# AmnonDrory/LidarRegistration

Hardware: AMD Instinct MI355X
Metric: registration pairs/sec (30k-pt FCGF pairs, mutual-NN + 50k RANSAC iters + refit) (higher is better)
Workload: dtype f32; 1 GPU; configs[1]: 30000-pt x32-d synthetic FCGF pair, --mode MNN --iters 50000, 3-pt sampling + ELC + LS refit; 192 distinct resident pairs per GPU, T copied to the host inside the timed region; pairs_per_batched_call=32, batched_calls_in_flight_per_gpu=2, parallelism=pair-sharded x1

## Files before the change

### lidarregistration_amd/csrc/lr_api.hip

```cpp
#include "lr_internal.h"
#include <stdarg.h>
#include <string.h>
#include <stdlib.h>
#include <new>

static thread_local char g_err[512] = "";

void lr_set_error(const char *fmt, ...)
{
    va_list ap;
    va_start(ap, fmt);
    vsnprintf(g_err, sizeof(g_err), fmt, ap);
    va_end(ap);
}

static_assert(sizeof(lr_ransac_params) == 72 && sizeof(lr_pair_params) == 112 && sizeof(lr_pair_result) == 496,
              "ABI structs changed: update include/lidarreg.h, _ext.py, INTEGRATION.md and tests/test_abi_cpu.py together");

extern "C" int lr_version(void) { return 103; }
extern "C" const char *lr_last_error(void) { return g_err; }

static inline void forget_last_batch(lr_workspace *ws) { if (ws) { ws->last_batch = 0; ws->last_T_final = nullptr; } }

static int g_fake_device = -1;
// ... 77 lines not shown
        T *p = base ? reinterpret_cast<T *>(base + off) : nullptr;
        off += sizeof(T) * count;
        return p;
    }
};

void carve(lr_workspace *ws, Carver &c)
{
    const size_t n0 = ws->max_n0, n1 = ws->max_n1, n = ws->max_n, it = ws->max_iters;
    ws->nrm0 = c.take<float>(n0); ws->nrm1 = c.take<float>(n1);
    ws->H0 = c.take<_Float16>(n0 * 32); ws->H1 = c.take<_Float16>(n1 * 32);
    if (ws->dim != LR_FEAT_DIM) { ws->P0 = c.take<float>(n0 * 32); ws->P1 = c.take<float>(n1 * 32); }
    ws->tau = c.take<float>(n);
    ws->yfin = c.take<float>(n * LR_NN_MAX_STRIPS);
    ws->yshare = c.take<uint32_t>(n);
    ws->cand_cnt = c.take<int32_t>(LR_NN16_CNT_INTS(n)); ws->cand = c.take<int32_t>(LR_NN16_SEG_INTS(n));
    ws->counters = c.take<int32_t>(LR_CNT_TOTAL);
    ws->bmax0 = c.take<float>(n0 / 32 + 2); ws->bmax1 = c.take<float>(n1 / 32 + 2);
    ws->bmin0 = c.take<float>(n0 / 32 + 2); ws->bmin1 = c.take<float>(n1 / 32 + 2);
    ws->nn_range = c.take<float>(8);
    ws->rev_seed = c.take<uint32_t>(n1); ws->rev_rows = c.take<int32_t>(n1);
    ws->rev_seed64 = c.take<unsigned long long>(n1);
    ws->rev_cols = c.take<int32_t>(n0); ws->rev_s1 = c.take<float>(n0); ws->rev_pos = c.take<int32_t>(n0);
    ws->rev_tmin = c.take<float>(n0 / 32 + 2); ws->rev_hist = c.take<int32_t>(2 * 4096);
    ws->Hs = c.take<_Float16>(n0 * 32); ws->nrms = c.take<float>(n0);
    ws->nn_idx1 = c.take<int32_t>(n0); ws->nn_idx2 = c.take<int32_t>(n0);
    ws->nn_s1 = c.take<float>(n0); ws->nn_s2 = c.take<float>(n0);
    ws->rev_idx1 = c.take<int32_t>(n1);
    ws->is_bb = c.take<uint8_t>(n0);
    ws->blk_cnt = c.take<int32_t>(n0 / 256 + 2);
    ws->corr_idx0 = c.take<int32_t>(n0); ws->corr_idx1 = c.take<int32_t>(n0); ws->corr_idx2 = c.take<int32_t>(n0);
    ws->corr_score = c.take<float>(n0);
    ws->ratio = c.take<float>(n0);
    ws->cell = c.take<int32_t>(n0); ws->cell_sorted = c.take<int32_t>(n0);
    ws->gpf_quota = c.take<double>(LR_GPF_MAX_CELLS);
    ws->gpf_cells = c.take<int32_t>(3 * (LR_GPF_MAX_CELLS + 8) > 2 * (LR_PR_BUCKETS + 8) + 8 ? 3 * (LR_GPF_MAX_CELLS + 8) : 2 * (LR_PR_BUCKETS + 8) + 8);
    ws->gpf_keep = c.take<uint8_t>(n0);
    ws->gpf_f = c.take<float>(8);
    ws->corr8 = c.take<float>((n0 + 2) * 8);
    ws->prosac_G = c.take<int32_t>(n0 + 2); ws->prosac_rank = c.take<int32_t>(n0);
    ws->models = c.take<float>(it * 12);
    ws->models64 = c.take<double>(it * 12);
    ws->model_h = c.take<int32_t>(it);
    ws->models2 = c.take<float>(it * 12); ws->models64_2 = c.take<double>(it * 12); ws->model_h2 = c.take<int32_t>(it);
    ws->score_cnt = c.take<uint32_t>(it);
    ws->score_ssq = c.take<unsigned long long>(it);
    ws->refit_part = c.take<double>((n0 / 256 + 2) * 16);
// ... 157 lines not shown
__global__ void __launch_bounds__(256) zero_scratch_kernel(uint32_t *__restrict__ p, size_t words, lr_zargs z)
{
    lr_z(p, z, blockIdx.z);
    for (size_t k = (size_t)blockIdx.x * 256 + threadIdx.x; k < words; k += (size_t)gridDim.x * 256) p[k] = 0u;
}
int lr_zero_scratch(const lr_call &c, void *p, size_t bytes)
{
    const size_t words = (bytes + 3) / 4;
    int blocks = (int)((words + 255) / 256);
    if (blocks > 1024) blocks = 1024;
    hipLaunchKernelGGL(zero_scratch_kernel, dim3(blocks < 1 ? 1 : blocks, 1, c.pairs), dim3(256), 0, c.st, reinterpret_cast<uint32_t *>(p), words, c.z);
    LR_LAUNCH_CHECK();
    return LR_OK;
}

extern "C" int lr_workspace_clock(lr_workspace *ws, double *mhz, unsigned long long *cycles, unsigned long long *ticks, int reset)
{
    LR_CHECK_DEVICE(ws, nullptr, "lr_workspace_clock");
    unsigned long long h[2] = { 0ull, 0ull };
    LR_HIP(hipMemcpy(h, ws->clk_dev, sizeof h, hipMemcpyDeviceToHost));
    if (cycles) *cycles = h[0];
    if (ticks) *ticks = h[1];
    if (mhz) *mhz = h[1] ? 100.0 * (double)h[0] / (double)h[1] : 0.0;
    if (reset) LR_HIP(hipMemset(ws->clk_dev, 0, sizeof h));
    return LR_OK;
}

int lr_timer_mark(const lr_call &c, lr_event e)
{
    lr_stage_timer &t = c.ws->timer;
    bool due = false;
    switch (e) {
    case LR_EV_FWD_FILTER_BEGIN: case LR_EV_FWD_FILTER_END: due = c.armed && !t.begun(); break;
    case LR_EV_REV_FILTER_BEGIN: case LR_EV_REV_FILTER_END: due = t.begun() && !t.has(LR_EV_REV_FILTER_END) && !t.has(LR_EV_RANSAC_END); break;
    case LR_EV_RANSAC_BEGIN: case LR_EV_RANSAC_END: due = t.begun() && !t.has(LR_EV_RANSAC_END); break;
    case LR_EV_CALL_BEGIN: case LR_EV_FWD_NN_DONE: case LR_EV_REV_NN_DONE: due = c.armed; break;
    case LR_EV_CALL_END: due = c.armed && t.has(LR_EV_RANSAC_END); break;
    case LR_NEV: break;
    }
    if (!t.on || !due) return LR_OK;
    LR_HIP(hipEventRecord(t.ev[e], c.st));
    t.recorded |= 1u << e;
    return LR_OK;
}

static int lr_timer_collect(lr_stage_timer &t)
{
// ... 359 lines not shown
```

### lidarregistration_amd/csrc/lr_internal.h

```cpp
#pragma once
#include <hip/hip_runtime.h>
#include <stdint.h>
#include <stdio.h>
#include "../../include/lidarreg.h"

void lr_set_error(const char *fmt, ...);

#define LR_HIP(call)                                                                      \
    do {                                                                                  \
        hipError_t e_ = (call);                                                           \
        if (e_ != hipSuccess) {                                                           \
            lr_set_error("%s:%d: %s -> %s", __FILE__, __LINE__, #call, hipGetErrorString(e_)); \
            return LR_EHIP;                                                               \
        }                                                                                 \
    } while (0)

#define LR_LAUNCH_CHECK() LR_HIP(hipGetLastError())

#define LR_REQUIRE(cond, code, msg)                 \
    do {                                            \
        if (!(cond)) { lr_set_error("%s", msg); return code; } \
    } while (0)

#define LR_NN16_SEG 4096
// ... 13 lines not shown
        } } while (0)

#define LR_NN_MAX_STRIPS 8
#define LR_FEAT_DIM 32

#ifndef LR_SCORE_BLOCKS
#define LR_SCORE_BLOCKS 2048
#endif
#define LR_GPF_MAX_CELLS 4096
#define LR_PR_BUCKETS 8192
#define LR_SC_INFO_BYTES 2048
#define LR_LO_CTL_BYTES 20480

struct lr_pair_desc {
    const float *xyz0, *xyz1, *F0, *F1;
    int32_t n0, n1;
};
struct lr_zargs {
    size_t stride;
    const lr_pair_desc *descs;
};
#define LR_MAX_BATCH 64
struct lr_desc_table { lr_pair_desc d[LR_MAX_BATCH]; };

#ifdef __HIPCC__
#define lr_z(p, z, pair) \
    do { const size_t lr_zo_ = (size_t)(pair) * (z).stride; p = (decltype(p))((const char *)(p) + (lr_zo_ & ((size_t)0 - (size_t)((p) != nullptr)))); } while (0)
__device__ __forceinline__ bool lr_xcd_block(int total, int &logical)
{
    const int chunk = (int)gridDim.x >> 3;
    logical = ((int)blockIdx.x & 7) * chunk + ((int)blockIdx.x >> 3);
    return logical < total;
}
#endif

enum lr_event {
    LR_EV_FWD_FILTER_BEGIN, LR_EV_FWD_FILTER_END,
    LR_EV_RANSAC_BEGIN, LR_EV_RANSAC_END,
    LR_EV_REV_FILTER_BEGIN, LR_EV_REV_FILTER_END,
    LR_EV_CALL_BEGIN,
    LR_EV_FWD_NN_DONE, LR_EV_CALL_END, LR_EV_REV_NN_DONE,
    LR_NEV
};
struct lr_stage_timer {
    int on;
    unsigned recorded;
// ... 16 lines not shown
    hipStream_t last_stream;
    size_t stride;
    size_t bytes;
    char *base;
    lr_pair_desc *descs;
    float *nrm0, *nrm1;
    _Float16 *H0, *H1;
    float *P0, *P1;
    float *tau;
    uint32_t *yshare;
    float *yfin;
    int32_t *cand_cnt, *cand;
    float *bmax0, *bmax1;
    float *bmin0, *bmin1;
    float *nn_range;
    int form_prev[2];
    int32_t *form_host, *form_dev;
    uint32_t *rev_seed;
    unsigned long long *rev_seed64;
    int32_t *rev_rows;
    int32_t *rev_cols;
    int32_t *rev_pos;
    float *rev_s1;
    float *rev_tmin;
    int32_t *rev_hist;
    _Float16 *Hs; float *nrms;
    int nn_blocks_target;
    int nn_blocks_batch;
    int nn_sample_stride;
    int rev_strips;
    int nn_second_auto;
    int clock_probe;
    unsigned long long *clk_dev;
    int32_t *counters;
    int32_t *nn_idx1, *nn_idx2;
    float *nn_s1, *nn_s2;
    int32_t *rev_idx1;
    uint8_t *is_bb;
    int32_t *blk_cnt;
    int32_t *corr_idx0, *corr_idx1, *corr_idx2;
    float *corr_score;
    float *ratio;
    int32_t *cell;
    int32_t *cell_sorted;
    double *gpf_quota;
    int32_t *gpf_cells;
    uint8_t *gpf_keep;
    float *gpf_f;
// ... 108 lines not shown
```

### lidarregistration_amd/csrc/lr_nn16.hip

```cpp
#include "lr_internal.h"
#include <math.h>
#include <stdlib.h>
#include <type_traits>

typedef float f32x4 __attribute__((ext_vector_type(4)));
typedef float f32x2 __attribute__((ext_vector_type(2)));
typedef _Float16 f16x8 __attribute__((ext_vector_type(8)));

#define LR_INF __builtin_huge_valf()
#define LR_IMAX 0x7fffffff

__device__ __forceinline__ uint32_t lr_ord_enc(float v) { const uint32_t b = __float_as_uint(v); return (b & 0x80000000u) ? ~b : (b | 0x80000000u); }
__device__ __forceinline__ float lr_ord_dec(uint32_t u) { return __uint_as_float((u & 0x80000000u) ? (u & 0x7fffffffu) : ~u); }
#define LR_ORD_INF 0xff800000u

__global__ void __launch_bounds__(256)
nn16_prep_kernel(const float *__restrict__ Fa, int na, _Float16 *__restrict__ Ha, float *__restrict__ nrma, float *__restrict__ bmaxa, float *__restrict__ bmina,
                 const float *__restrict__ Fb, int nb, _Float16 *__restrict__ Hb, float *__restrict__ nrmb, float *__restrict__ bmaxb, float *__restrict__ bminb,
                 uint32_t *__restrict__ seed_b, unsigned long long *__restrict__ seed64_b, int32_t *__restrict__ counters, int zero_counters, int nblk_a,
                 uint32_t *__restrict__ yshare_a, lr_zargs z)
{
    __shared__ float s_m[4], s_n[4];
    if (z.descs) { const lr_pair_desc d = z.descs[blockIdx.z]; Fa = d.F0; na = d.n0; Fb = d.F1; nb = d.n1; }
    lr_z(bmina, z, blockIdx.z); lr_z(bminb, z, blockIdx.z);
    lr_z(Ha, z, blockIdx.z); lr_z(nrma, z, blockIdx.z); lr_z(bmaxa, z, blockIdx.z); lr_z(Hb, z, blockIdx.z); lr_z(nrmb, z, blockIdx.z);
    lr_z(bmaxb, z, blockIdx.z); lr_z(seed_b, z, blockIdx.z); lr_z(seed64_b, z, blockIdx.z); lr_z(counters, z, blockIdx.z); lr_z(yshare_a, z, blockIdx.z);
    if (counters && blockIdx.x == 0 && (int)threadIdx.x < LR_CNT_TOTAL) {
        const int k = threadIdx.x;
// ... 158 lines not shown
        atomicMin(&o.seed_range[0], __float_as_uint(lo));
        atomicMax(&o.seed_range[1], __float_as_uint(hi));
    }
}
__device__ __forceinline__ bool ex_bad8(const f32x4 &u, const f32x4 &v)
{
    const float big = fmaxf(fmaxf(fmaxf(fabsf(u.x), fabsf(u.y)), fmaxf(fabsf(u.z), fabsf(u.w))), fmaxf(fmaxf(fabsf(v.x), fabsf(v.y)), fmaxf(fabsf(v.z), fabsf(v.w))));
    return !(big <= 65504.0f) || u.x != u.x || u.y != u.y || u.z != u.z || u.w != u.w || v.x != v.x || v.y != v.y || v.z != v.z || v.w != v.w;
}

#ifdef LR_PB_PROBE
__device__ unsigned long long lr_pb_stat[16];
#define LR_PROBE(...) __VA_ARGS__
#else
#define LR_PROBE(...)
#endif
#define LR_PB_WAVES 3
template <bool SIGN>
__global__ void __launch_bounds__(256) __attribute__((amdgpu_waves_per_eu(LR_PB_WAVES, LR_PB_WAVES)))
nn16_passb_kernel(lr_pb_tail tail_first , unsigned long long *clk_on,
                  const _Float16 *__restrict__ Hq, int na_host, const int32_t *__restrict__ rowmap, const int32_t *__restrict__ na_dev,
                  const _Float16 *__restrict__ Hc, const float *__restrict__ nC, int nb,
                  int tiles_per_strip, const float *__restrict__ tau, int32_t *__restrict__ cand_cnt, int32_t *__restrict__ cand,
                  const int32_t *__restrict__ colmap, const float *__restrict__ tile_min, const uint32_t *__restrict__ row_bound,
                  const int32_t *__restrict__ rev_offs, const uint32_t *__restrict__ rev_range, float *__restrict__ yfin, int yfin_stride,
                  uint32_t *__restrict__ yshare, int32_t *__restrict__ form_miss, lr_thr_in thr, lr_pb_grid pg, lr_zargs z)
{
    int logical;
    if (!lr_xcd_block(pg.total, logical)) return;
    const int bx = logical % pg.gx, by = (logical / pg.gx) % pg.gy, pair = logical / (pg.gx * pg.gy);
    if (z.descs) {
        const lr_pair_desc d = z.descs[pair];
        na_host = pg.dir ? d.n1 : d.n0; nb = pg.dir ? d.n0 : d.n1;
    }
    lr_z(Hq, z, pair); lr_z(rowmap, z, pair); lr_z(na_dev, z, pair); lr_z(Hc, z, pair); lr_z(nC, z, pair); lr_z(tau, z, pair);
    lr_z(cand_cnt, z, pair); lr_z(cand, z, pair); lr_z(colmap, z, pair); lr_z(tile_min, z, pair); lr_z(row_bound, z, pair); lr_z(rev_offs, z, pair); lr_z(rev_range, z, pair);
    lr_z(thr.nQ, z, pair); lr_z(thr.range_c, z, pair); lr_z(yfin, z, pair); lr_z(yshare, z, pair);
    const int na = na_dev ? *na_dev : na_host;
    if (bx * LR_BLOCK_ROWS >= na) return;
    float max_nc = 0.0f, min_nc = 0.0f;
    if (thr.range_c) { max_nc = thr.range_c[0]; min_nc = thr.range_c[1]; }
    const bool sign_ok = thr.range_c != nullptr && min_nc > 0.0f && max_nc < LR_INF && max_nc - min_nc <= 1e-4f * max_nc && true;
    if (sign_ok != SIGN) {
        if (pg.only && form_miss && bx == 0 && by == 0 && threadIdx.x == 0) { lr_z(form_miss, z, pair); *form_miss = 1; }
        return;
    }
    const float xhat = SIGN ? 0.5f * min_nc : 0.0f;
    __shared__ int s_limit[4];
    __shared__ unsigned long long s_clk[2];
    if (clk_on && threadIdx.x == 0) { s_clk[0] = __builtin_amdgcn_s_memtime(); s_clk[1] = __builtin_amdgcn_s_memrealtime(); }
    constexpr int CH = LR_PB_CH;
    constexpr int XOFF = CH * 32 * LR_LDS_ROW;
    constexpr int BUF = XOFF + (SIGN ? 0 : CH * 32 * 4);
    __shared__ __attribute__((aligned(16))) unsigned char lds_a[BUF];
    __shared__ __attribute__((aligned(16))) unsigned char lds_b[BUF];
    constexpr int WL = (LR_PB_CH >= 8 && !SIGN) ? (LR_PB_WLIST * 7) / 8 : LR_PB_WLIST;
    __shared__ uint2 wlist[4][WL];
    __shared__ __attribute__((aligned(16))) float s_Y[LR_BLOCK_ROWS];
    __shared__ float s_D[LR_BLOCK_ROWS], s_N1[LR_BLOCK_ROWS], s_N2[LR_BLOCK_ROWS];
    __shared__ unsigned s_att[2];
    const int tid = threadIdx.x, wave = __builtin_amdgcn_readfirstlane(tid >> 6), lane = tid & 63;
    const int c16 = lane & 15, kb = lane >> 4;
    const int row0 = bx * LR_BLOCK_ROWS + wave * 64;
    LR_PROBE(int n_visits = 0, n_hits = 0, n_rounds = 0, n_groups = 0, n_tk_derive = 0, n_tk_flush = 0, n_tk_a = 0, n_tk_b = 0;
             const unsigned long long tk_start = __builtin_amdgcn_s_memrealtime(); unsigned long long tk_walk = 0;)
    int ntiles = (nb + 31) >> 5;
    int my_strips = pg.gy;
    if (tile_min) {
        if (tid == 0) {
            const float lo = __uint_as_float(rev_range[0]), scale = rs_scale(lo, __uint_as_float(rev_range[1]));
            const float sv = __uint_as_float(row_bound[rowmap[bx * LR_BLOCK_ROWS]]);
            const int b = rs_bucket(sv, lo, scale);
            s_limit[0] = ((b + 1 < LR_RS_BUCKETS ? rev_offs[b + 1] : nb) + 31) >> 5;
        }
        __syncthreads();
        ntiles = min(ntiles, s_limit[0]);
        my_strips = min(pg.gy, (ntiles + tiles_per_strip - 1) / tiles_per_strip);
        if (by >= my_strips) return;
        tiles_per_strip = (ntiles + my_strips - 1) / my_strips;
    }
    const int t_begin = by * tiles_per_strip;
    const int t_end = min(ntiles, t_begin + tiles_per_strip);
    const int nchunks = t_end > t_begin ? (t_end - t_begin + CH - 1) / CH : 0;

    f16x8 a16[4];
#pragma unroll
    for (int rbk = 0; rbk < 4; ++rbk) {
        int row = min(row0 + 16 * rbk + c16, na - 1);
        if (rowmap) row = rowmap[row];
        a16[rbk] = *reinterpret_cast<const f16x8 *>(Hq + (size_t)row * 32 + 8 * kb);
    }

    f32x4 stage[CH / 2];
    float stage_n = 0.0f;

    {
        const int rw = bx * LR_BLOCK_ROWS + tid;
        float Dv = LR_INF;
        if (thr.nQ && rw < na) {
// ... 582 lines not shown
    lr_workspace *ws = c.ws;
    hipLaunchKernelGGL(nn16_prep_kernel, dim3(lr_cdiv(n0, 32) + lr_cdiv(n1, 32), 1, c.pairs), dim3(256), 0, c.st, F0, n0, ws->H0, ws->nrm0, ws->bmax0, ws->bmin0,
                       F1, n1, ws->H1, ws->nrm1, ws->bmax1, ws->bmin1, ws->rev_seed, ws->rev_seed64, ws->counters, zero_counters ? 1 : 0, lr_cdiv(n0, 32), ws->yshare, c.z);
    hipLaunchKernelGGL(nn16_range_kernel, dim3(2, 1, c.pairs), dim3(256), 0, c.st, n0, (const float *)ws->bmax0, (const float *)ws->bmin0, n1, (const float *)ws->bmax1,
                       (const float *)ws->bmin1, ws->nn_range, c.pairs == 1 ? ws->form_dev : (int32_t *)nullptr, c.z);
    LR_LAUNCH_CHECK();
    return LR_OK;
}

static int lr_nn16_form_hint(const lr_call &c, int col_cloud)
{
    lr_workspace *ws = c.ws;
    if (c.pairs != 1 || !ws->form_host) return 0;
    const int h = *reinterpret_cast<const volatile int32_t *>(&ws->form_host[col_cloud]);
    const int prev = ws->form_prev[col_cloud];
    ws->form_prev[col_cloud] = h;
    return ((h == 1 || h == 2) && h == prev) ? h : 0;
}

struct lr_pb_args {
    const _Float16 *Hq; int na; const int32_t *rowmap, *na_dev;
    const _Float16 *Hc; const float *nC; int nb, tps;
    const float *tau;
    const int32_t *colmap; const float *tile_min; const uint32_t *row_bound; const int32_t *rev_offs; const uint32_t *rev_range;
    float *yfin; int yfin_stride; uint32_t *yshare;
    lr_thr_in thr;
    int row_blocks, strips, dir;
};
static int lr_nn16_passb(const lr_call &c, const lr_pb_args &a)
{
    lr_workspace *ws = c.ws;
    const int total = a.row_blocks * a.strips * c.pairs;
    const dim3 grid(8 * lr_cdiv(total, 8));
    LR_TRY_HIP(lr_timer_mark(c, a.dir ? LR_EV_REV_FILTER_BEGIN : LR_EV_FWD_FILTER_BEGIN));
    const int only = lr_nn16_form_hint(c, a.dir ? 0 : 1);
    int32_t *miss = ws->counters + (a.dir ? LR_CNT_FORM_MISS_R : LR_CNT_FORM_MISS_F);
    unsigned long long *clk = ws->clock_probe ? ws->clk_dev : (unsigned long long *)nullptr;
    const lr_pb_tail tl = { clk };
    const lr_pb_grid pg = { a.row_blocks, a.strips, total, a.dir, only };
    auto launch = [&](auto kernel) {
        hipLaunchKernelGGL(kernel, grid, dim3(256), 0, c.st, tl, clk, a.Hq, a.na, a.rowmap, a.na_dev, a.Hc, a.nC, a.nb, a.tps, a.tau, ws->cand_cnt, ws->cand,
                           a.colmap, a.tile_min, a.row_bound, a.rev_offs, a.rev_range, a.yfin, a.yfin_stride, a.yshare, miss, a.thr, pg, c.z);
    };
    if (only != 2) launch(nn16_passb_kernel<true>);
    if (only != 1) launch(nn16_passb_kernel<false>);
    return lr_timer_mark(c, a.dir ? LR_EV_REV_FILTER_END : LR_EV_FWD_FILTER_END);
}

int lr_nn16_run(const lr_call &c, const float *Fq, int na, const float *Fc, int nb,
                int32_t *idx1, int32_t *idx2, float *s1, float *s2, bool seed_reverse)
{
    lr_workspace *ws = c.ws;
    const float *nQ = ws->nrm0, *nC = ws->nrm1, *range_c = ws->nn_range + 2;
    const int need = idx2 ? 2 : 1;
    const int ntiles = lr_cdiv(nb, 32);
    const int row_blocks = lr_cdiv(na, LR_BLOCK_ROWS);
    int strips = c.pairs > 1 ? lr_cdiv(ws->nn_blocks_batch, row_blocks * c.pairs) : ws->nn_blocks_target / row_blocks;
    int smax = ntiles / 64;
    if (strips > smax) strips = smax;
    if (strips > LR_NN_MAX_STRIPS) strips = LR_NN_MAX_STRIPS;
    if (strips < 1) strips = 1;
    const int tps = lr_cdiv(ntiles, strips);
    int sstride = ws->nn_sample_stride > 0 ? ws->nn_sample_stride : (strips > 1 ? ntiles / 64 : tps / 32);
    if (ws->nn_sample_stride <= 0) { const int cap = strips > 1 ? 16 : 32; if (sstride > cap) sstride = cap; }
    if (sstride < 1) sstride = 1;
// ... 32 lines not shown
        const f32x4 a = pa[k], b = pb[k];
        acc = __builtin_fmaf(a.x, b.x, acc);
        acc = __builtin_fmaf(a.y, b.y, acc);
        acc = __builtin_fmaf(a.z, b.z, acc);
        acc = __builtin_fmaf(a.w, b.w, acc);
    }
    const float d2 = __builtin_fmaf(-2.0f, acc, n0v[i] + n1v[j]);
    sv = __builtin_sqrtf(fmaxf(d2, 1e-30f));
    if (!(sv < 3.0e38f)) sv = 3.0e38f;
    atomicMin(&seed_bits[j], __float_as_uint(sv));
    s1[i] = sv;
    }
    float lo = i < n0 ? sv : 3.0e38f, hi = i < n0 ? sv : 0.0f;
#pragma unroll
    for (int k = 32; k >= 1; k >>= 1) { lo = fminf(lo, __shfl_xor(lo, k)); hi = fmaxf(hi, __shfl_xor(hi, k)); }
    if ((threadIdx.x & 63) == 0) { s_lo[threadIdx.x >> 6] = lo; s_hi[threadIdx.x >> 6] = hi; }
    __syncthreads();
    if (threadIdx.x == 0) {
        atomicMin(&range[0], __float_as_uint(fminf(fminf(s_lo[0], s_lo[1]), fminf(s_lo[2], s_lo[3]))));
        atomicMax(&range[1], __float_as_uint(fmaxf(fmaxf(s_hi[0], s_hi[1]), fmaxf(s_hi[2], s_hi[3]))));
    }
}

#define LR_RO_ROUND 8192
#define LR_RO_QUEUE 3072
__global__ void __launch_bounds__(1024)
nn16_rev_order_kernel(int n0, int n1, const float *__restrict__ s1, const uint32_t *__restrict__ seed_bits, const uint32_t *__restrict__ range,
                      int32_t *__restrict__ offs, int32_t *__restrict__ n_rows, const float *__restrict__ block_max_c, int nblk_c,
                      const float *__restrict__ nrm1, const _Float16 *__restrict__ H0, const float *__restrict__ nrm0, int32_t *__restrict__ colmap,
                      _Float16 *__restrict__ H0s, float *__restrict__ nrm0s, int32_t *__restrict__ rowmap, float *__restrict__ tau,
                      int32_t *__restrict__ cand_cnt, int32_t *__restrict__ rev_out, int seg_counters, lr_zargs z)
{
    __shared__ int s_pos[2 * LR_RS_BUCKETS];
    __shared__ int2 s_q[LR_RO_QUEUE];
    __shared__ float s_m[16];
    __shared__ int s_w[16], s_own[4], s_nq, s_nrows;
    if (z.descs) { n0 = z.descs[blockIdx.z].n0; n1 = z.descs[blockIdx.z].n1; nblk_c = (n0 + 31) >> 5; }
    lr_z(s1, z, blockIdx.z); lr_z(seed_bits, z, blockIdx.z); lr_z(range, z, blockIdx.z); lr_z(offs, z, blockIdx.z); lr_z(n_rows, z, blockIdx.z);
    lr_z(block_max_c, z, blockIdx.z); lr_z(nrm1, z, blockIdx.z); lr_z(H0, z, blockIdx.z); lr_z(nrm0, z, blockIdx.z); lr_z(colmap, z, blockIdx.z);
    lr_z(H0s, z, blockIdx.z); lr_z(nrm0s, z, blockIdx.z); lr_z(rowmap, z, blockIdx.z); lr_z(tau, z, blockIdx.z); lr_z(cand_cnt, z, blockIdx.z); lr_z(rev_out, z, blockIdx.z);
    const int tid = threadIdx.x, lane = tid & 63, part = blockIdx.x, parts = gridDim.x;
    for (int k = part * 1024 + tid; k < seg_counters; k += parts * 1024) cand_cnt[k] = 0;
    const float lo = __uint_as_float(range[0]), scale = rs_scale(lo, __uint_as_float(range[1]));
    for (int k = tid; k < 2 * LR_RS_BUCKETS; k += 1024) s_pos[k] = 0;
    if (tid < 4) s_own[tid] = (tid & 1) ? 0 : 0x7fffffff;
    if (tid == 0) s_nq = 0;
    float mx = 0.0f;
    for (int b = tid; b < nblk_c; b += 1024) mx = fmaxf(mx, block_max_c[b]);
#pragma unroll
    for (int k = 32; k >= 1; k >>= 1) mx = fmaxf(mx, __shfl_xor(mx, k));
    if (lane == 0) s_m[tid >> 6] = mx;
    __syncthreads();
    float max_nc = 0.0f;
#pragma unroll
    for (int w = 0; w < 16; ++w) max_nc = fmaxf(max_nc, s_m[w]);
    for (int i0 = tid; i0 < max(n0, n1); i0 += 8 * 1024) {
        float v[8]; uint32_t u[8];
#pragma unroll
        for (int k = 0; k < 8; ++k) { v[k] = s1[min(i0 + 1024 * k, n0 - 1)]; u[k] = seed_bits[min(i0 + 1024 * k, n1 - 1)]; }
#pragma unroll
        for (int k = 0; k < 8; ++k) {
            if (i0 + 1024 * k < n0) atomicAdd(&s_pos[rs_bucket(v[k], lo, scale)], 1);
            const float sv = __uint_as_float(u[k]);
            if (i0 + 1024 * k < n1 && sv <= 3.0e38f) atomicAdd(&s_pos[LR_RS_BUCKETS + (LR_RS_BUCKETS - 1 - rs_bucket(sv, lo, scale))], 1);
        }
    }
    __syncthreads();
    for (int side = 0; side < 2; ++side) {
        int *hp = s_pos + side * LR_RS_BUCKETS;
        int v[LR_RS_BUCKETS / 1024], sum = 0;
#pragma unroll
        for (int k = 0; k < LR_RS_BUCKETS / 1024; ++k) { v[k] = hp[tid * (LR_RS_BUCKETS / 1024) + k]; sum += v[k]; }
        int inc = sum;
#pragma unroll
        for (int d = 1; d < 64; d <<= 1) { const int o = __shfl_up(inc, d); if (lane >= d) inc += o; }
        if (lane == 63) s_w[tid >> 6] = inc;
        __syncthreads();
        int base = 0;
        for (int w = 0; w < (tid >> 6); ++w) base += s_w[w];
        int run = base + inc - sum;
#pragma unroll
        for (int k = 0; k < LR_RS_BUCKETS / 1024; ++k) {
            hp[tid * (LR_RS_BUCKETS / 1024) + k] = run;
            if (part == 0) offs[side * LR_RS_BUCKETS + tid * (LR_RS_BUCKETS / 1024) + k] = run;
            run += v[k];
        }
        if (side == 1 && tid == 1023) { s_nrows = run; if (part == 0) *n_rows = run; }
        __syncthreads();
    }
    {
        const long long nrows = s_nrows;
        for (int k = tid; k < 2 * LR_RS_BUCKETS; k += 1024) {
            const int side = k >= LR_RS_BUCKETS, kb = k & (LR_RS_BUCKETS - 1);
            const long long n = side ? nrows : (long long)n0, lo_p = (long long)part * n, hi_p = (long long)(part + 1) * n;
            auto own = [&](int idx) { const long long sp = (long long)s_pos[idx] * parts; return sp >= lo_p && sp < hi_p; };
            if (own(k)) {
                if (kb == 0 || !own(k - 1)) s_own[2 * side] = k;
                if (kb == LR_RS_BUCKETS - 1 || !own(k + 1)) s_own[2 * side + 1] = k + 1;
            }
        }
    }
    __syncthreads();
    const int c_lo = s_own[0], c_len = max(s_own[1] - s_own[0], 0), r_lo = s_own[2], r_len = max(s_own[3] - s_own[2], 0);
    constexpr int U = LR_RO_ROUND / 1024;
    auto move_row = [&](int i, int p, int piece) {
        reinterpret_cast<f32x4 *>(H0s + (size_t)p * 32)[piece] = reinterpret_cast<const f32x4 *>(H0 + (size_t)i * 32)[piece];
        if (piece == 0) { colmap[p] = i; nrm0s[p] = nrm0[i]; }
    };
    for (int i0 = 0; i0 < n0; i0 += LR_RO_ROUND) {
        float v[U];
#pragma unroll
        for (int k = 0; k < U; ++k) v[k] = s1[min(i0 + tid + 1024 * k, n0 - 1)];
#pragma unroll
        for (int k = 0; k < U; ++k) {
            const int i = i0 + tid + 1024 * k, b = rs_bucket(v[k], lo, scale);
            if (i < n0 && (unsigned)(b - c_lo) < (unsigned)c_len) {
                const int p = atomicAdd(&s_pos[b], 1), slot = atomicAdd(&s_nq, 1);
                if (slot < LR_RO_QUEUE) s_q[slot] = make_int2(i, p);
                else { for (int piece = 0; piece < 4; ++piece) move_row(i, p, piece); }
            }
        }
        __syncthreads();
        const int nq = min(s_nq, LR_RO_QUEUE);
        __syncthreads();
// ... 7 lines not shown
#pragma unroll
        for (int k = 0; k < U1; ++k) v[k] = seed_bits[min(j0 + 1024 * k, n1 - 1)];
#pragma unroll
        for (int k = 0; k < U1; ++k) {
            const int row = j0 + 1024 * k;
            if (row >= n1) continue;
            const float sv = __uint_as_float(v[k]);
            if (!(sv <= 3.0e38f)) {
                if ((row & (parts - 1)) == part) rev_out[row] = -1;
                continue;
            }
            const int b = LR_RS_BUCKETS + (LR_RS_BUCKETS - 1 - rs_bucket(sv, lo, scale));
            if ((unsigned)(b - r_lo) >= (unsigned)r_len) continue;
            const int p = atomicAdd(&s_pos[b], 1);
            const float nj = nrm1[row], scl = nj + max_nc;
            const float E = 1.05e-3f * scl + 4e-7f;
            const float d2hi = sv * sv * (1.0f + 6e-7f);
            rowmap[p] = row;
            tau[p] = (d2hi - nj) + E + 6e-6f * scl + 2e-6f * d2hi;
        }
    }
}

int lr_nn16_reverse(const lr_call &c, const float *F0, int n0, const float *F1, int n1, const int32_t *fwd_idx1, int32_t *rev, bool seeded)
{
    lr_workspace *ws = c.ws; hipStream_t st = c.st;
    const float *nrm0 = ws->nrm0, *nrm1 = ws->nrm1;
    const int na = n1, nb = n0;
    const int ntiles = lr_cdiv(nb, 32);
    const int row_blocks = lr_cdiv(na, LR_BLOCK_ROWS);
    int strips = ws->rev_strips > 0 ? ws->rev_strips : 48 / c.pairs;
    if (ws->rev_strips <= 0) { if (strips > 8) strips = 8; if (strips < 2) strips = 2; }
    int smax = ntiles / 8;
    if (strips > smax) strips = smax;
    if (strips < 1) strips = 1;
    const int tps = lr_cdiv(ntiles, strips);
    uint32_t *seed = ws->rev_seed;
    uint32_t *range = reinterpret_cast<uint32_t *>(ws->counters + LR_CNT_RLO);
    int32_t *n_rows = ws->counters + LR_CNT_NREV;
    if (!seeded)
        hipLaunchKernelGGL(nn16_rev_seed_kernel, dim3(lr_cdiv(n0, 256)), dim3(256), 0, st, F0, nrm0, n0, F1, nrm1, fwd_idx1, seed, ws->rev_s1, range);
    const int order_parts = c.pairs >= 16 ? 8 : c.pairs >= 4 ? 16 : 32;
    hipLaunchKernelGGL(nn16_rev_order_kernel, dim3(order_parts, 1, c.pairs), dim3(1024), 0, st, n0, n1, (const float *)ws->rev_s1, (const uint32_t *)seed,
                       (const uint32_t *)range, ws->rev_hist, n_rows, (const float *)ws->bmax0, lr_cdiv(nb, 32), nrm1, (const _Float16 *)ws->H0, nrm0, ws->rev_cols, ws->Hs, ws->nrms,
                       ws->rev_rows, ws->tau, ws->cand_cnt, rev, row_blocks * 4 * (strips + 1), c.z);
    lr_pb_args a = {};
    a.Hq = ws->H1; a.na = na; a.rowmap = ws->rev_rows; a.na_dev = n_rows; a.Hc = ws->Hs; a.nC = ws->nrms; a.nb = nb; a.tps = tps;
    a.tau = ws->tau;
    a.colmap = ws->rev_cols; a.tile_min = seeded ? ws->rev_tmin : nullptr; a.row_bound = seed; a.rev_offs = ws->rev_hist; a.rev_range = range;
    a.thr = lr_thr_in{ nullptr, ws->nn_range, 1, 0 };
    a.row_blocks = row_blocks; a.strips = strips; a.dir = 1;
    LR_TRY_HIP(lr_nn16_passb(c, a));
    const lr_ex_out reo = { rev, nullptr, nullptr, nullptr, nullptr, nullptr, nullptr, seeded ? ws->rev_seed64 : (unsigned long long *)nullptr };
    const int ex_gx = lr_cdiv(na, LR_EX_ROWS), ex_total = ex_gx * c.pairs;
    hipLaunchKernelGGL(nn16_exact_kernel, dim3(8 * lr_cdiv(ex_total, 8)), dim3(256), 0, st, F1, nrm1, na, F0, nrm0, nb, ws->cand_cnt, ws->cand,
                       strips, 1, (const float *)nullptr, 0, (const int32_t *)ws->rev_rows, (const int32_t *)n_rows, reo, ws->counters,
                       (const float *)ws->nn_range, 1, ex_gx, ex_total, c.z);
    LR_LAUNCH_CHECK();
    return LR_OK;
}
```

Before: 12520 pairs/s.

## Split reverse ordering into hist/scan/move kernels and precompute per-block tile limits

For batches of 16 or more pairs, the single reverse-order kernel (in which each part rescanned all data) is replaced by three kernels. Per-slice histograms are built first, then one block per pair scans them into per-slice offsets, then each slice scatters its own rows and columns. Per-row-block tile limits are also precomputed, so the pass-B kernel reads one int per block instead of doing a bucket lookup and a barrier. The cost is two extra launches and a partition table in global memory. A stream synchronize is also added to the clock reset.

```diff
diff --git a/lidarregistration_amd/csrc/lr_api.hip b/lidarregistration_amd/csrc/lr_api.hip
--- a/lidarregistration_amd/csrc/lr_api.hip
+++ b/lidarregistration_amd/csrc/lr_api.hip
@@ -123,7 +123,7 @@
     ws->rev_seed = c.take<uint32_t>(n1); ws->rev_rows = c.take<int32_t>(n1);
     ws->rev_seed64 = c.take<unsigned long long>(n1);
     ws->rev_cols = c.take<int32_t>(n0); ws->rev_s1 = c.take<float>(n0); ws->rev_pos = c.take<int32_t>(n0);
-    ws->rev_tmin = c.take<float>(n0 / 32 + 2); ws->rev_hist = c.take<int32_t>(2 * 4096);
+    ws->rev_lim = c.take<int32_t>(n1 / 256 + 2); ws->rev_part = c.take<int32_t>(LR_RO_PARTS * 2 * 4096);
     ws->Hs = c.take<_Float16>(n0 * 32); ws->nrms = c.take<float>(n0);
     ws->nn_idx1 = c.take<int32_t>(n0); ws->nn_idx2 = c.take<int32_t>(n0);
     ws->nn_s1 = c.take<float>(n0); ws->nn_s2 = c.take<float>(n0);
@@ -327,7 +327,10 @@
     if (cycles) *cycles = h[0];
     if (ticks) *ticks = h[1];
     if (mhz) *mhz = h[1] ? 100.0 * (double)h[0] / (double)h[1] : 0.0;
-    if (reset) LR_HIP(hipMemset(ws->clk_dev, 0, sizeof h));
+    if (reset) {
+        LR_HIP(hipMemset(ws->clk_dev, 0, sizeof h));
+        LR_HIP(hipStreamSynchronize(nullptr));
+    }
     return LR_OK;
 }
 
diff --git a/lidarregistration_amd/csrc/lr_internal.h b/lidarregistration_amd/csrc/lr_internal.h
--- a/lidarregistration_amd/csrc/lr_internal.h
+++ b/lidarregistration_amd/csrc/lr_internal.h
@@ -59,6 +59,7 @@
 };
 #define LR_MAX_BATCH 64
 struct lr_desc_table { lr_pair_desc d[LR_MAX_BATCH]; };
+#define LR_RO_PARTS 8
 
 #ifdef __HIPCC__
 #define lr_z(p, z, pair) \
@@ -121,8 +122,8 @@
     int32_t *rev_cols;
     int32_t *rev_pos;
     float *rev_s1;
-    float *rev_tmin;
-    int32_t *rev_hist;
+    int32_t *rev_lim;
+    int32_t *rev_part;
     _Float16 *Hs; float *nrms;
     int nn_blocks_target;
     int nn_blocks_batch;
diff --git a/lidarregistration_amd/csrc/lr_nn16.hip b/lidarregistration_amd/csrc/lr_nn16.hip
--- a/lidarregistration_amd/csrc/lr_nn16.hip
+++ b/lidarregistration_amd/csrc/lr_nn16.hip
@@ -4,6 +4,7 @@
 #include <type_traits>
 
 typedef float f32x4 __attribute__((ext_vector_type(4)));
+typedef int i32x4 __attribute__((ext_vector_type(4)));
 typedef float f32x2 __attribute__((ext_vector_type(2)));
 typedef _Float16 f16x8 __attribute__((ext_vector_type(8)));
 
@@ -208,8 +209,7 @@
                   const _Float16 *__restrict__ Hq, int na_host, const int32_t *__restrict__ rowmap, const int32_t *__restrict__ na_dev,
                   const _Float16 *__restrict__ Hc, const float *__restrict__ nC, int nb,
                   int tiles_per_strip, const float *__restrict__ tau, int32_t *__restrict__ cand_cnt, int32_t *__restrict__ cand,
-                  const int32_t *__restrict__ colmap, const float *__restrict__ tile_min, const uint32_t *__restrict__ row_bound,
-                  const int32_t *__restrict__ rev_offs, const uint32_t *__restrict__ rev_range, float *__restrict__ yfin, int yfin_stride,
+                  const int32_t *__restrict__ colmap, const int32_t *__restrict__ tile_lim, float *__restrict__ yfin, int yfin_stride,
                   uint32_t *__restrict__ yshare, int32_t *__restrict__ form_miss, lr_thr_in thr, lr_pb_grid pg, lr_zargs z)
 {
     int logical;
@@ -220,7 +220,7 @@
         na_host = pg.dir ? d.n1 : d.n0; nb = pg.dir ? d.n0 : d.n1;
     }
     lr_z(Hq, z, pair); lr_z(rowmap, z, pair); lr_z(na_dev, z, pair); lr_z(Hc, z, pair); lr_z(nC, z, pair); lr_z(tau, z, pair);
-    lr_z(cand_cnt, z, pair); lr_z(cand, z, pair); lr_z(colmap, z, pair); lr_z(tile_min, z, pair); lr_z(row_bound, z, pair); lr_z(rev_offs, z, pair); lr_z(rev_range, z, pair);
+    lr_z(cand_cnt, z, pair); lr_z(cand, z, pair); lr_z(colmap, z, pair); lr_z(tile_lim, z, pair);
     lr_z(thr.nQ, z, pair); lr_z(thr.range_c, z, pair); lr_z(yfin, z, pair); lr_z(yshare, z, pair);
     const int na = na_dev ? *na_dev : na_host;
     if (bx * LR_BLOCK_ROWS >= na) return;
@@ -232,7 +232,6 @@
         return;
     }
     const float xhat = SIGN ? 0.5f * min_nc : 0.0f;
-    __shared__ int s_limit[4];
     __shared__ unsigned long long s_clk[2];
     if (clk_on && threadIdx.x == 0) { s_clk[0] = __builtin_amdgcn_s_memtime(); s_clk[1] = __builtin_amdgcn_s_memrealtime(); }
     constexpr int CH = LR_PB_CH;
@@ -252,15 +251,8 @@
              const unsigned long long tk_start = __builtin_amdgcn_s_memrealtime(); unsigned long long tk_walk = 0;)
     int ntiles = (nb + 31) >> 5;
     int my_strips = pg.gy;
-    if (tile_min) {
-        if (tid == 0) {
-            const float lo = __uint_as_float(rev_range[0]), scale = rs_scale(lo, __uint_as_float(rev_range[1]));
-            const float sv = __uint_as_float(row_bound[rowmap[bx * LR_BLOCK_ROWS]]);
-            const int b = rs_bucket(sv, lo, scale);
-            s_limit[0] = ((b + 1 < LR_RS_BUCKETS ? rev_offs[b + 1] : nb) + 31) >> 5;
-        }
-        __syncthreads();
-        ntiles = min(ntiles, s_limit[0]);
+    if (tile_lim) {
+        ntiles = min(ntiles, tile_lim[bx]);
         my_strips = min(pg.gy, (ntiles + tiles_per_strip - 1) / tiles_per_strip);
         if (by >= my_strips) return;
         tiles_per_strip = (ntiles + my_strips - 1) / my_strips;
@@ -889,7 +881,7 @@
     const _Float16 *Hq; int na; const int32_t *rowmap, *na_dev;
     const _Float16 *Hc; const float *nC; int nb, tps;
     const float *tau;
-    const int32_t *colmap; const float *tile_min; const uint32_t *row_bound; const int32_t *rev_offs; const uint32_t *rev_range;
+    const int32_t *colmap, *tile_lim;
     float *yfin; int yfin_stride; uint32_t *yshare;
     lr_thr_in thr;
     int row_blocks, strips, dir;
@@ -907,7 +899,7 @@
     const lr_pb_grid pg = { a.row_blocks, a.strips, total, a.dir, only };
     auto launch = [&](auto kernel) {
         hipLaunchKernelGGL(kernel, grid, dim3(256), 0, c.st, tl, clk, a.Hq, a.na, a.rowmap, a.na_dev, a.Hc, a.nC, a.nb, a.tps, a.tau, ws->cand_cnt, ws->cand,
-                           a.colmap, a.tile_min, a.row_bound, a.rev_offs, a.rev_range, a.yfin, a.yfin_stride, a.yshare, miss, a.thr, pg, c.z);
+                           a.colmap, a.tile_lim, a.yfin, a.yfin_stride, a.yshare, miss, a.thr, pg, c.z);
     };
     if (only != 2) launch(nn16_passb_kernel<true>);
     if (only != 1) launch(nn16_passb_kernel<false>);
@@ -986,11 +978,22 @@
     }
 }
 
+__device__ __forceinline__ void ro_write_prefix(const int *s_pos, int n_rows, int nb, int32_t *__restrict__ tile_lim)
+{
+    for (int k = threadIdx.x; k < LR_RS_BUCKETS; k += 1024) {
+        const int start = s_pos[LR_RS_BUCKETS + k], end = k + 1 < LR_RS_BUCKETS ? s_pos[LR_RS_BUCKETS + k + 1] : n_rows;
+        if (end <= start) continue;
+        const int b = LR_RS_BUCKETS - 1 - k;
+        const int lim = ((b + 1 < LR_RS_BUCKETS ? s_pos[b + 1] : nb) + 31) >> 5;
+        for (int bx = (start + LR_BLOCK_ROWS - 1) / LR_BLOCK_ROWS; bx * LR_BLOCK_ROWS < end; ++bx) tile_lim[bx] = lim;
+    }
+}
+
 #define LR_RO_ROUND 8192
 #define LR_RO_QUEUE 3072
 __global__ void __launch_bounds__(1024)
 nn16_rev_order_kernel(int n0, int n1, const float *__restrict__ s1, const uint32_t *__restrict__ seed_bits, const uint32_t *__restrict__ range,
-                      int32_t *__restrict__ offs, int32_t *__restrict__ n_rows, const float *__restrict__ block_max_c, int nblk_c,
+                      int32_t *__restrict__ tile_lim, int32_t *__restrict__ n_rows, const float *__restrict__ block_max_c, int nblk_c,
                       const float *__restrict__ nrm1, const _Float16 *__restrict__ H0, const float *__restrict__ nrm0, int32_t *__restrict__ colmap,
                       _Float16 *__restrict__ H0s, float *__restrict__ nrm0s, int32_t *__restrict__ rowmap, float *__restrict__ tau,
                       int32_t *__restrict__ cand_cnt, int32_t *__restrict__ rev_out, int seg_counters, lr_zargs z)
@@ -1000,7 +1003,7 @@
     __shared__ float s_m[16];
     __shared__ int s_w[16], s_own[4], s_nq, s_nrows;
     if (z.descs) { n0 = z.descs[blockIdx.z].n0; n1 = z.descs[blockIdx.z].n1; nblk_c = (n0 + 31) >> 5; }
-    lr_z(s1, z, blockIdx.z); lr_z(seed_bits, z, blockIdx.z); lr_z(range, z, blockIdx.z); lr_z(offs, z, blockIdx.z); lr_z(n_rows, z, blockIdx.z);
+    lr_z(s1, z, blockIdx.z); lr_z(seed_bits, z, blockIdx.z); lr_z(range, z, blockIdx.z); lr_z(tile_lim, z, blockIdx.z); lr_z(n_rows, z, blockIdx.z);
     lr_z(block_max_c, z, blockIdx.z); lr_z(nrm1, z, blockIdx.z); lr_z(H0, z, blockIdx.z); lr_z(nrm0, z, blockIdx.z); lr_z(colmap, z, blockIdx.z);
     lr_z(H0s, z, blockIdx.z); lr_z(nrm0s, z, blockIdx.z); lr_z(rowmap, z, blockIdx.z); lr_z(tau, z, blockIdx.z); lr_z(cand_cnt, z, blockIdx.z); lr_z(rev_out, z, blockIdx.z);
     const int tid = threadIdx.x, lane = tid & 63, part = blockIdx.x, parts = gridDim.x;
@@ -1046,7 +1049,6 @@
 #pragma unroll
         for (int k = 0; k < LR_RS_BUCKETS / 1024; ++k) {
             hp[tid * (LR_RS_BUCKETS / 1024) + k] = run;
-            if (part == 0) offs[side * LR_RS_BUCKETS + tid * (LR_RS_BUCKETS / 1024) + k] = run;
             run += v[k];
         }
         if (side == 1 && tid == 1023) { s_nrows = run; if (part == 0) *n_rows = run; }
@@ -1064,6 +1066,7 @@
             }
         }
     }
+    if (part == 0) ro_write_prefix(s_pos, s_nrows, n0, tile_lim);
     __syncthreads();
     const int c_lo = s_own[0], c_len = max(s_own[1] - s_own[0], 0), r_lo = s_own[2], r_len = max(s_own[3] - s_own[2], 0);
     constexpr int U = LR_RO_ROUND / 1024;
@@ -1117,6 +1120,153 @@
     }
 }
 
+#define LR_RO_SLICED_PAIRS 16
+#define LR_RO_SROUND 4096
+__device__ __forceinline__ int ro_slice(int n, int q) { return (int)((long long)q * n / LR_RO_PARTS); }
+
+__global__ void __launch_bounds__(1024)
+nn16_ro_hist_kernel(int n0, int n1, const float *__restrict__ s1, const uint32_t *__restrict__ seed_bits, const uint32_t *__restrict__ range,
+                    int32_t *__restrict__ table, lr_zargs z)
+{
+    __shared__ __attribute__((aligned(16))) int s_h[2 * LR_RS_BUCKETS];
+    if (z.descs) { n0 = z.descs[blockIdx.z].n0; n1 = z.descs[blockIdx.z].n1; }
+    lr_z(s1, z, blockIdx.z); lr_z(seed_bits, z, blockIdx.z); lr_z(range, z, blockIdx.z); lr_z(table, z, blockIdx.z);
+    const int tid = threadIdx.x, part = blockIdx.x;
+    const float lo = __uint_as_float(range[0]), scale = rs_scale(lo, __uint_as_float(range[1]));
+    for (int k = tid; k < 2 * LR_RS_BUCKETS; k += 1024) s_h[k] = 0;
+    __syncthreads();
+    const int c0 = ro_slice(n0, part), c1 = ro_slice(n0, part + 1), r0 = ro_slice(n1, part), r1 = ro_slice(n1, part + 1);
+    for (int i0 = c0 + tid; i0 < c1; i0 += 4 * 1024) {
+        float v[4];
+#pragma unroll
+        for (int k = 0; k < 4; ++k) v[k] = s1[min(i0 + 1024 * k, c1 - 1)];
+#pragma unroll
+        for (int k = 0; k < 4; ++k)
+            if (i0 + 1024 * k < c1) atomicAdd(&s_h[rs_bucket(v[k], lo, scale)], 1);
+    }
+    for (int j0 = r0 + tid; j0 < r1; j0 += 4 * 1024) {
+        uint32_t u[4];
+#pragma unroll
+        for (int k = 0; k < 4; ++k) u[k] = seed_bits[min(j0 + 1024 * k, r1 - 1)];
+#pragma unroll
+        for (int k = 0; k < 4; ++k) {
+            const float sv = __uint_as_float(u[k]);
+            if (j0 + 1024 * k < r1 && sv <= 3.0e38f) atomicAdd(&s_h[LR_RS_BUCKETS + (LR_RS_BUCKETS - 1 - rs_bucket(sv, lo, scale))], 1);
+        }
+    }
+    __syncthreads();
+    i32x4 *out = reinterpret_cast<i32x4 *>(table + (size_t)part * 2 * LR_RS_BUCKETS);
+    for (int k = tid; k < 2 * LR_RS_BUCKETS / 4; k += 1024) out[k] = reinterpret_cast<const i32x4 *>(s_h)[k];
+}
+
+__global__ void __launch_bounds__(1024)
+nn16_ro_scan_kernel(int n0, int32_t *__restrict__ table, int32_t *__restrict__ n_rows, int32_t *__restrict__ tile_lim,
+                    int32_t *__restrict__ cand_cnt, int seg_counters, lr_zargs z)
+{
+    static_assert(LR_RS_BUCKETS == 4 * 1024, "four buckets per thread, one 16-byte word of every table row");
+    __shared__ int s_pos[2 * LR_RS_BUCKETS];
+    __shared__ int s_w[16], s_nrows;
+    if (z.descs) n0 = z.descs[blockIdx.z].n0;
+    lr_z(table, z, blockIdx.z); lr_z(n_rows, z, blockIdx.z); lr_z(tile_lim, z, blockIdx.z); lr_z(cand_cnt, z, blockIdx.z);
+    const int tid = threadIdx.x, lane = tid & 63;
+    for (int k = tid; k < seg_counters; k += 1024) cand_cnt[k] = 0;
+    for (int side = 0; side < 2; ++side) {
+        i32x4 *col = reinterpret_cast<i32x4 *>(table) + side * 1024 + tid;
+        i32x4 c[LR_RO_PARTS];
+#pragma unroll
+        for (int q = 0; q < LR_RO_PARTS; ++q) c[q] = col[q * (2 * LR_RS_BUCKETS / 4)];
+        i32x4 tot = c[0];
+#pragma unroll
+        for (int q = 1; q < LR_RO_PARTS; ++q) tot += c[q];
+        const int sum = tot.x + tot.y + tot.z + tot.w;
+        int inc = sum;
+#pragma unroll
+        for (int d = 1; d < 64; d <<= 1) { const int o = __shfl_up(inc, d); if (lane >= d) inc += o; }
+        if (lane == 63) s_w[tid >> 6] = inc;
+        __syncthreads();
+        int base = 0;
+        for (int w = 0; w < (tid >> 6); ++w) base += s_w[w];
+        i32x4 run;
+        run.x = base + inc - sum; run.y = run.x + tot.x; run.z = run.y + tot.y; run.w = run.z + tot.z;
+        int *hp = s_pos + side * LR_RS_BUCKETS + 4 * tid;
+        hp[0] = run.x; hp[1] = run.y; hp[2] = run.z; hp[3] = run.w;
+#pragma unroll
+        for (int q = 0; q < LR_RO_PARTS; ++q) { col[q * (2 * LR_RS_BUCKETS / 4)] = run; run += c[q]; }
+        if (side == 1 && tid == 1023) { s_nrows = base + inc; *n_rows = base + inc; }
+        __syncthreads();
+    }
+    ro_write_prefix(s_pos, s_nrows, n0, tile_lim);
+}
+
+__global__ void __launch_bounds__(1024)
+nn16_ro_move_kernel(int n0, int n1, const float *__restrict__ s1, const uint32_t *__restrict__ seed_bits, const uint32_t *__restrict__ range,
+                    const int32_t *__restrict__ table, const float *__restrict__ block_max_c, int nblk_c,
+                    const float *__restrict__ nrm1, const _Float16 *__restrict__ H0, const float *__restrict__ nrm0, int32_t *__restrict__ colmap,
+                    _Float16 *__restrict__ H0s, float *__restrict__ nrm0s, int32_t *__restrict__ rowmap, float *__restrict__ tau,
+                    int32_t *__restrict__ rev_out, lr_zargs z)
+{
+    __shared__ __attribute__((aligned(16))) int s_pos[2 * LR_RS_BUCKETS];
+    __shared__ int s_p[LR_RO_SROUND];
+    __shared__ float s_m[16];
+    if (z.descs) { n0 = z.descs[blockIdx.z].n0; n1 = z.descs[blockIdx.z].n1; nblk_c = (n0 + 31) >> 5; }
+    lr_z(s1, z, blockIdx.z); lr_z(seed_bits, z, blockIdx.z); lr_z(range, z, blockIdx.z); lr_z(table, z, blockIdx.z);
+    lr_z(block_max_c, z, blockIdx.z); lr_z(nrm1, z, blockIdx.z); lr_z(H0, z, blockIdx.z); lr_z(nrm0, z, blockIdx.z); lr_z(colmap, z, blockIdx.z);
+    lr_z(H0s, z, blockIdx.z); lr_z(nrm0s, z, blockIdx.z); lr_z(rowmap, z, blockIdx.z); lr_z(tau, z, blockIdx.z); lr_z(rev_out, z, blockIdx.z);
+    const int tid = threadIdx.x, lane = tid & 63, part = blockIdx.x;
+    const float lo = __uint_as_float(range[0]), scale = rs_scale(lo, __uint_as_float(range[1]));
+    {
+        const i32x4 *in = reinterpret_cast<const i32x4 *>(table + (size_t)part * 2 * LR_RS_BUCKETS);
+        for (int k = tid; k < 2 * LR_RS_BUCKETS / 4; k += 1024) reinterpret_cast<i32x4 *>(s_pos)[k] = in[k];
+    }
+    float mx = 0.0f;
+    for (int b = tid; b < nblk_c; b += 1024) mx = fmaxf(mx, block_max_c[b]);
+#pragma unroll
+    for (int k = 32; k >= 1; k >>= 1) mx = fmaxf(mx, __shfl_xor(mx, k));
+    if (lane == 0) s_m[tid >> 6] = mx;
+    __syncthreads();
+    float max_nc = 0.0f;
+#pragma unroll
+    for (int w = 0; w < 16; ++w) max_nc = fmaxf(max_nc, s_m[w]);
+    const int c0 = ro_slice(n0, part), c1 = ro_slice(n0, part + 1), r0 = ro_slice(n1, part), r1 = ro_slice(n1, part + 1);
+    constexpr int U = LR_RO_SROUND / 1024;
+    for (int i0 = c0; i0 < c1; i0 += LR_RO_SROUND) {
+        float v[U];
+#pragma unroll
+        for (int k = 0; k < U; ++k) v[k] = s1[min(i0 + tid + 1024 * k, c1 - 1)];
+#pragma unroll
+        for (int k = 0; k < U; ++k)
+            if (i0 + tid + 1024 * k < c1) s_p[tid + 1024 * k] = atomicAdd(&s_pos[rs_bucket(v[k], lo, scale)], 1);
+        __syncthreads();
+        const int cnt = min(LR_RO_SROUND, c1 - i0), piece = tid & 3;
+#pragma unroll 4
+        for (int e = tid >> 2; e < cnt; e += 256) {
+            const int i = i0 + e, p = s_p[e];
+            reinterpret_cast<f32x4 *>(H0s + (size_t)p * 32)[piece] = reinterpret_cast<const f32x4 *>(H0 + (size_t)i * 32)[piece];
+            if (piece == 0) { colmap[p] = i; nrm0s[p] = nrm0[i]; }
+        }
+        __syncthreads();
+    }
+    for (int j0 = r0 + tid; j0 < r1; j0 += U * 1024) {
+        uint32_t v[U];
+#pragma unroll
+        for (int k = 0; k < U; ++k) v[k] = seed_bits[min(j0 + 1024 * k, r1 - 1)];
+#pragma unroll
+        for (int k = 0; k < U; ++k) {
+            const int row = j0 + 1024 * k;
+            if (row >= r1) continue;
+            const float sv = __uint_as_float(v[k]);
+            if (!(sv <= 3.0e38f)) { rev_out[row] = -1; continue; }
+            const int b = LR_RS_BUCKETS + (LR_RS_BUCKETS - 1 - rs_bucket(sv, lo, scale));
+            const int p = atomicAdd(&s_pos[b], 1);
+            const float nj = nrm1[row], scl = nj + max_nc;
+            const float E = 1.05e-3f * scl + 4e-7f;
+            const float d2hi = sv * sv * (1.0f + 6e-7f);
+            rowmap[p] = row;
+            tau[p] = (d2hi - nj) + E + 6e-6f * scl + 2e-6f * d2hi;
+        }
+    }
+}
+
 int lr_nn16_reverse(const lr_call &c, const float *F0, int n0, const float *F1, int n1, const int32_t *fwd_idx1, int32_t *rev, bool seeded)
 {
     lr_workspace *ws = c.ws; hipStream_t st = c.st;
@@ -1135,14 +1285,24 @@
     int32_t *n_rows = ws->counters + LR_CNT_NREV;
     if (!seeded)
         hipLaunchKernelGGL(nn16_rev_seed_kernel, dim3(lr_cdiv(n0, 256)), dim3(256), 0, st, F0, nrm0, n0, F1, nrm1, fwd_idx1, seed, ws->rev_s1, range);
-    const int order_parts = c.pairs >= 16 ? 8 : c.pairs >= 4 ? 16 : 32;
-    hipLaunchKernelGGL(nn16_rev_order_kernel, dim3(order_parts, 1, c.pairs), dim3(1024), 0, st, n0, n1, (const float *)ws->rev_s1, (const uint32_t *)seed,
-                       (const uint32_t *)range, ws->rev_hist, n_rows, (const float *)ws->bmax0, lr_cdiv(nb, 32), nrm1, (const _Float16 *)ws->H0, nrm0, ws->rev_cols, ws->Hs, ws->nrms,
-                       ws->rev_rows, ws->tau, ws->cand_cnt, rev, row_blocks * 4 * (strips + 1), c.z);
+    const int seg_counters = row_blocks * 4 * (strips + 1);
+    if (c.pairs >= LR_RO_SLICED_PAIRS) {
+        hipLaunchKernelGGL(nn16_ro_hist_kernel, dim3(LR_RO_PARTS, 1, c.pairs), dim3(1024), 0, st, n0, n1, (const float *)ws->rev_s1, (const uint32_t *)seed,
+                           (const uint32_t *)range, ws->rev_part, c.z);
+        hipLaunchKernelGGL(nn16_ro_scan_kernel, dim3(1, 1, c.pairs), dim3(1024), 0, st, n0, ws->rev_part, n_rows, ws->rev_lim, ws->cand_cnt, seg_counters, c.z);
+        hipLaunchKernelGGL(nn16_ro_move_kernel, dim3(LR_RO_PARTS, 1, c.pairs), dim3(1024), 0, st, n0, n1, (const float *)ws->rev_s1, (const uint32_t *)seed,
+                           (const uint32_t *)range, (const int32_t *)ws->rev_part, (const float *)ws->bmax0, lr_cdiv(nb, 32), nrm1, (const _Float16 *)ws->H0, nrm0,
+                           ws->rev_cols, ws->Hs, ws->nrms, ws->rev_rows, ws->tau, rev, c.z);
+    } else {
+        const int order_parts = c.pairs >= 4 ? 16 : 32;
+        hipLaunchKernelGGL(nn16_rev_order_kernel, dim3(order_parts, 1, c.pairs), dim3(1024), 0, st, n0, n1, (const float *)ws->rev_s1, (const uint32_t *)seed,
+                           (const uint32_t *)range, ws->rev_lim, n_rows, (const float *)ws->bmax0, lr_cdiv(nb, 32), nrm1, (const _Float16 *)ws->H0, nrm0, ws->rev_cols, ws->Hs, ws->nrms,
+                           ws->rev_rows, ws->tau, ws->cand_cnt, rev, seg_counters, c.z);
+    }
     lr_pb_args a = {};
     a.Hq = ws->H1; a.na = na; a.rowmap = ws->rev_rows; a.na_dev = n_rows; a.Hc = ws->Hs; a.nC = ws->nrms; a.nb = nb; a.tps = tps;
     a.tau = ws->tau;
-    a.colmap = ws->rev_cols; a.tile_min = seeded ? ws->rev_tmin : nullptr; a.row_bound = seed; a.rev_offs = ws->rev_hist; a.rev_range = range;
+    a.colmap = ws->rev_cols; a.tile_lim = seeded ? ws->rev_lim : nullptr;
     a.thr = lr_thr_in{ nullptr, ws->nn_range, 1, 0 };
     a.row_blocks = row_blocks; a.strips = strips; a.dir = 1;
     LR_TRY_HIP(lr_nn16_passb(c, a));
```

Result: slower. 12070 pairs/s (-3.6%).
